# robertknight/ocrs

Hardware: AMD Instinct MI355X
Metric: pages/sec end-to-end (1024x1024) (higher is better)
Workload: dtype f32

## Files before the change

### include/ocrs_amd.h

```cpp
#ifndef OCRS_AMD_H
#define OCRS_AMD_H

#include <stddef.h>
#include <stdint.h>

#if defined(__GNUC__)
#define OCRS_API __attribute__((visibility("default")))
#else
#define OCRS_API
#endif

#ifdef __cplusplus
extern "C" {
#endif

typedef enum ocrs_status {
    OCRS_OK = 0,
    OCRS_ERR_INVALID_ARGUMENT = 1,
    OCRS_ERR_MODEL_NOT_LOADED = 2,
    OCRS_ERR_MODEL_DIMS = 3,
    OCRS_ERR_RUN_FAILED = 4,
    OCRS_ERR_WRONG_OUTPUT = 5,
    OCRS_ERR_IMAGE_SOURCE = 6,
    OCRS_ERR_DEVICE = 7,
    OCRS_ERR_IO = 8,
    OCRS_ERR_CAPACITY = 9
} ocrs_status;

OCRS_API const char* ocrs_last_error(void);

#define OCRS_ABI_VERSION 6u
OCRS_API uint32_t ocrs_abi_version(void);

OCRS_API void ocrs_buffer_free(void* p);

OCRS_API ocrs_status ocrs_device_count(int* n);
OCRS_API ocrs_status ocrs_set_device(int device);
OCRS_API ocrs_status ocrs_get_device(int* device);

OCRS_API ocrs_status ocrs_ctc_beam_search(const float* logp, int t, int c, uint32_t width, int impl, uint32_t** labels,
                                          uint32_t** positions, size_t* n);
OCRS_API ocrs_status ocrs_ctc_beam_search_scored(const float* logp, int t, int c, uint32_t width, int impl, uint32_t** labels,
                                                 uint32_t** positions, size_t* n, double* score, float** step_logp);

OCRS_API ocrs_status ocrs_ctc_decode_packed(const float* logits, const int32_t* lengths, size_t n, int c, const uint8_t* excluded,
                                            int method, uint32_t width, uint32_t** labels, uint32_t** positions,
                                            size_t* step_offsets, float** step_logp, double* scores, float** logp);

OCRS_API ocrs_status ocrs_mask_component_rects(const uint8_t* masks, size_t n, int h, int w, float expand, float min_area,
                                               int max_comp, int64_t arena, int32_t* n_roots, int32_t* overflow, float* rects,
                                               uint8_t* valid);

OCRS_API ocrs_status ocrs_gru_tile_plan(const int32_t* lengths_desc, size_t n_lines, int hidden, int32_t* n_clusters, int32_t* waves,
                                        int16_t* tiles);

OCRS_API ocrs_status ocrs_coalescer_selftest(int n_threads, int requests_per_thread, int max_active, int max_pages,
                                             long window_us, int fail_every, uint64_t out[5]);

OCRS_API ocrs_status ocrs_stream_plan_selftest(int budget, const int32_t* ops, size_t n_ops, int32_t* out);

OCRS_API ocrs_status ocrs_conv_rows_selftest(const float* w, size_t n_w, const float* bias, size_t n_bias, int relu, int y0, int h,
                                             int cin, int32_t out[6]);

OCRS_API ocrs_status ocrs_set_option(const char* name, long value);
OCRS_API ocrs_status ocrs_option_name(int index, const char** name);

OCRS_API ocrs_status ocrs_device_pool_stats(int device, uint64_t out[12]);
OCRS_API ocrs_status ocrs_device_pool_configure(int device, uint64_t device_cached_cap_bytes, uint64_t pinned_cached_cap_bytes);
OCRS_API ocrs_status ocrs_device_pool_trim(int device);

typedef enum { OCRS_ISOLATION_AUTO = 0, OCRS_ISOLATION_NONE = 1 } ocrs_isolation;
OCRS_API ocrs_status ocrs_device_set_isolation(int device, ocrs_isolation policy);
OCRS_API ocrs_status ocrs_device_isolation(int device, int out[3]);

typedef struct ocrs_model ocrs_model;

OCRS_API ocrs_status ocrs_model_load_file(const char* path, ocrs_model** out);
OCRS_API ocrs_status ocrs_model_load_bytes(const void* data, size_t len, ocrs_model** out);
OCRS_API ocrs_status ocrs_model_load_file_on_device(const char* path, int device, ocrs_model** out);
OCRS_API ocrs_status ocrs_model_load_bytes_on_device(const void* data, size_t len, int device, ocrs_model** out);
OCRS_API ocrs_status ocrs_model_device(const ocrs_model* m, int* device);

typedef int (*ocrs_model_run_fn)(void* user, const float* input, const int64_t in_shape[4], float** output,
                                 int64_t out_shape[4], int* out_ndim);
OCRS_API ocrs_status ocrs_model_from_callback(const int64_t input_shape[4],
                                     ocrs_model_run_fn run, void* user, ocrs_model** out);

OCRS_API ocrs_status ocrs_model_input_shape(const ocrs_model* m, int64_t dims[4], uint8_t is_fixed[4]);

typedef struct ocrs_run_options {
    int timing;
} ocrs_run_options;

OCRS_API ocrs_status ocrs_model_run(const ocrs_model* m, const float* input, const int64_t in_shape[4],
                           const ocrs_run_options* opts, float** output, int64_t out_shape[4], int* out_ndim);

OCRS_API ocrs_status ocrs_model_flops(const ocrs_model* m, const int64_t in_shape[4], double* flops);

OCRS_API void ocrs_model_free(ocrs_model* m);

typedef struct ocrs_engine ocrs_engine;
typedef struct ocrs_page ocrs_page;

typedef enum ocrs_numerics { OCRS_NUMERICS_EXACT = 0, OCRS_NUMERICS_RELAXED = 1, OCRS_NUMERICS_REDUCED = 2 } ocrs_numerics;

typedef enum ocrs_decode_method {
    OCRS_DECODE_GREEDY = 0,
    OCRS_DECODE_BEAM_SEARCH = 1
} ocrs_decode_method;

typedef struct ocrs_engine_params {
    const ocrs_model* detection_model;
    const ocrs_model* recognition_model;
    int debug;
    ocrs_decode_method decode_method;
    uint32_t beam_width;
    const char* alphabet;
    const char* allowed_chars;
    ocrs_numerics numerics;
    int coalesce;
    int coalesce_pages;
    int coalesce_window_us;
    int layout_threads;
    int64_t rec_max_pixels;
} ocrs_engine_params;

OCRS_API ocrs_status ocrs_engine_new(const ocrs_engine_params* params, ocrs_engine** out);
OCRS_API void ocrs_engine_free(ocrs_engine* e);
OCRS_API ocrs_status ocrs_engine_device(const ocrs_engine* e, int* device);
OCRS_API ocrs_status ocrs_engine_set_option(ocrs_engine* e, const char* name, long value);
OCRS_API ocrs_status ocrs_engine_get_option(const ocrs_engine* e, const char* name, long* value);

typedef enum ocrs_dim_order { OCRS_HWC = 0, OCRS_CHW = 1 } ocrs_dim_order;
typedef enum ocrs_pixel_type { OCRS_U8 = 0, OCRS_F32 = 1 } ocrs_pixel_type;

OCRS_API ocrs_status ocrs_image_source_check_bytes(size_t len, uint32_t width, uint32_t height, uint32_t* channels);

OCRS_API ocrs_status ocrs_engine_prepare_input(const ocrs_engine* e, const void* pixels, ocrs_pixel_type type,
                                      ocrs_dim_order order, int height, int width, int channels,
                                      ocrs_page** out);
OCRS_API ocrs_status ocrs_engine_prepare_input_batch(const ocrs_engine* e, const void* const* pixels, size_t n,
                                                     ocrs_pixel_type type, ocrs_dim_order order, int height, int width,
                                                     int channels, ocrs_page** out);
OCRS_API ocrs_status ocrs_engine_prepare_input_device(const ocrs_engine* e, const void* d_pixels, ocrs_pixel_type type,
                                             ocrs_dim_order order, int height, int width, int channels,
// ... 381 lines not shown
```

### ocrs_amd/_lib.py

```python
import ctypes as C
import os

_HERE = os.path.dirname(os.path.abspath(__file__))
LIB_PATH = os.environ.get("OCRS_AMD_LIB") or os.path.join(_HERE, "libocrs_amd.so")

OCRS_OK = 0
STATUS_NAMES = {
    0: "OK", 1: "INVALID_ARGUMENT", 2: "MODEL_NOT_LOADED", 3: "MODEL_DIMS", 4: "RUN_FAILED", 5: "WRONG_OUTPUT",
    6: "IMAGE_SOURCE", 7: "DEVICE", 8: "IO", 9: "CAPACITY",
}

RUN_FN = C.CFUNCTYPE(C.c_int, C.c_void_p, C.POINTER(C.c_float), C.POINTER(C.c_int64), C.POINTER(C.POINTER(C.c_float)),
                     C.POINTER(C.c_int64), C.POINTER(C.c_int))


class EngineParams(C.Structure):
    _fields_ = [("detection_model", C.c_void_p), ("recognition_model", C.c_void_p), ("debug", C.c_int),
                ("decode_method", C.c_int), ("beam_width", C.c_uint32), ("alphabet", C.c_char_p),
                ("allowed_chars", C.c_char_p), ("numerics", C.c_int), ("coalesce", C.c_int), ("coalesce_pages", C.c_int),
                ("coalesce_window_us", C.c_int), ("layout_threads", C.c_int), ("rec_max_pixels", C.c_int64)]


class GroupParams(C.Structure):
    _fields_ = [("detection_model", C.c_void_p), ("detection_model_len", C.c_size_t), ("recognition_model", C.c_void_p),
                ("recognition_model_len", C.c_size_t), ("devices", C.POINTER(C.c_int)), ("n_devices", C.c_size_t),
                ("debug", C.c_int), ("decode_method", C.c_int), ("beam_width", C.c_uint32), ("alphabet", C.c_char_p),
                ("allowed_chars", C.c_char_p), ("gather", C.c_int), ("numerics", C.c_int), ("coalesce", C.c_int),
                ("coalesce_pages", C.c_int), ("coalesce_window_us", C.c_int), ("layout_threads", C.c_int), ("rec_max_pixels", C.c_int64),
                ("min_block", C.c_int), ("shared_block", C.c_int)]


class RunOptions(C.Structure):
    _fields_ = [("timing", C.c_int)]


class TextCharC(C.Structure):
    _fields_ = [("ch", C.c_uint32), ("top", C.c_int32), ("left", C.c_int32), ("bottom", C.c_int32),
                ("right", C.c_int32)]


class OcrsError(RuntimeError):
    def __init__(self, status, message):
        super().__init__(message)
        self.status = status
        self.status_name = STATUS_NAMES.get(status, str(status))


DECLARED_SYMBOLS = [
    "ocrs_last_error", "ocrs_buffer_free", "ocrs_device_count", "ocrs_set_device", "ocrs_set_option", "ocrs_ctc_beam_search", "ocrs_model_load_file",
    "ocrs_model_load_bytes", "ocrs_model_from_callback", "ocrs_model_input_shape", "ocrs_model_run",
    "ocrs_model_flops", "ocrs_model_free", "ocrs_engine_new", "ocrs_engine_free", "ocrs_image_source_check_bytes",
    "ocrs_engine_prepare_input", "ocrs_engine_prepare_input_device", "ocrs_page_free", "ocrs_page_dims",
    "ocrs_page_image", "ocrs_engine_detect_words", "ocrs_engine_detect_words_batch",
    "ocrs_engine_detect_text_pixels", "ocrs_engine_detection_threshold", "ocrs_engine_find_text_lines",
    "ocrs_engine_find_text_lines_batch",
    "ocrs_engine_recognize_text", "ocrs_engine_recognize_text_batch", "ocrs_engine_recognize_tokens",
    "ocrs_engine_prepare_recognition_input", "ocrs_text_item_rotated_rect", "ocrs_rotated_rect_corners", "ocrs_engine_get_text", "ocrs_device_malloc", "ocrs_device_free",
    "ocrs_device_upload", "ocrs_device_synchronize", "ocrs_device_measure_peaks", "ocrs_engine_enable_timing", "ocrs_stage_count",
    "ocrs_stage_name", "ocrs_engine_stage_times", "ocrs_kernel_class_count", "ocrs_kernel_class_name",
    "ocrs_engine_kernel_stats", "ocrs_engine_set_kernel_timing_mask", "ocrs_gru_tile_plan", "ocrs_host_malloc", "ocrs_host_free", "ocrs_engine_prepare_input_batch",
    "ocrs_get_device", "ocrs_model_load_file_on_device", "ocrs_model_load_bytes_on_device", "ocrs_model_device", "ocrs_engine_device",
    "ocrs_engine_group_new", "ocrs_engine_group_free", "ocrs_engine_group_size", "ocrs_engine_group_member", "ocrs_group_deal",
    "ocrs_group_prepare_input_batch", "ocrs_group_prepare_input_device_batch", "ocrs_group_detect_words_batch",
    "ocrs_group_recognize_text_batch", "ocrs_group_gather", "ocrs_group_final_gather", "ocrs_group_worker_threads", "ocrs_group_last_gather", "ocrs_device_malloc_on", "ocrs_engine_coalesce_stats", "ocrs_coalescer_selftest", "ocrs_stream_plan_selftest", "ocrs_conv_rows_selftest", "ocrs_engine_kernel_mfma_flops", "ocrs_engine_prepare_input_jpeg", "ocrs_jpeg_decode_rgb", "ocrs_jpeg_info", "ocrs_jpeg_coefficients",
    "ocrs_group_member_stats", "ocrs_numa_parse_cpulist", "ocrs_numa_bind_selftest", "ocrs_engine_recognize_logits", "ocrs_engine_set_option", "ocrs_engine_get_option", "ocrs_option_name", "ocrs_device_pool_stats", "ocrs_device_pool_configure", "ocrs_device_pool_trim",
    "ocrs_device_set_isolation", "ocrs_device_isolation", "ocrs_group_set_replay", "ocrs_abi_version",
    "ocrs_engine_recognize_text_scored", "ocrs_engine_recognize_text_batch_scored", "ocrs_ctc_beam_search_scored",
    "ocrs_engine_run_recognition_ops", "ocrs_ctc_decode_packed", "ocrs_mask_component_rects",
    "ocrs_engine_detect_words_scored", "ocrs_engine_detect_words_batch_scored", "ocrs_group_detect_words_batch_scored",
    "ocrs_engine_find_text_lines_indexed", "ocrs_engine_find_text_lines_batch_indexed",
    "ocrs_detection_tile_plan", "ocrs_engine_detect_words_tiled", "ocrs_engine_detect_words_batch_tiled",
    "ocrs_engine_detect_text_pixels_tiled", "ocrs_group_detect_words_batch_tiled",
    "ocrs_line_frame", "ocrs_line_char_boxes", "ocrs_engine_prepare_recognition_input_rectified",
    "ocrs_engine_recognize_text_rectified", "ocrs_engine_recognize_text_batch_rectified",
    "ocrs_group_recognize_text_batch_rectified", "ocrs_engine_recognize_tokens_rectified",
    "ocrs_engine_rotate_page", "ocrs_engine_rotate_pages", "ocrs_unrotate_rects", "ocrs_unrotate_chars",
    "ocrs_orientation_vote", "ocrs_engine_detect_orientation", "ocrs_engine_page_from_grey",
    "ocrs_engine_resize_page", "ocrs_engine_resize_pages", "ocrs_work_size", "ocrs_rescale_rects",
    "ocrs_engine_detect_words_at", "ocrs_engine_detect_words_batch_at",
    "ocrs_normalize_params_default", "ocrs_normalize_params_check", "ocrs_engine_normalize_page", "ocrs_engine_normalize_pages",
    "ocrs_skew_params_default", "ocrs_skew_params_check", "ocrs_skew_table", "ocrs_engine_skew_scores", "ocrs_engine_estimate_skew",
    "ocrs_engine_warp_page", "ocrs_engine_warp_pages", "ocrs_deskew_map", "ocrs_unwarp_rects", "ocrs_unwarp_chars",
    "ocrs_outline_params_default", "ocrs_outline_params_check", "ocrs_engine_edge_peaks", "ocrs_outline_choose", "ocrs_engine_find_outline",
    "ocrs_quad_map", "ocrs_engine_project_page", "ocrs_engine_project_pages", "ocrs_unproject_rects", "ocrs_unproject_chars",
    "ocrs_rules_params_default", "ocrs_rules_params_check", "ocrs_engine_remove_rules_page", "ocrs_engine_remove_rules_pages",
    "ocrs_speckle_params_default", "ocrs_speckle_params_check", "ocrs_engine_despeckle_page", "ocrs_engine_despeckle_pages",
    "ocrs_binarize_params_default", "ocrs_binarize_params_check", "ocrs_engine_binarize_page", "ocrs_engine_binarize_pages",
]

ABI_VERSION = 6
TILE_OVERLAP_DEFAULT = 100
RESAMPLE_FILTERS = {"auto": 0, "bilinear": 1, "area": 2}
POLARITIES = {"auto": 0, "keep": 1, "invert": 2}


class NormalizeParams(C.Structure):
    _fields_ = [("tile", C.c_int32), ("polarity", C.c_int32), ("flatten", C.c_int32), ("levels", C.c_int32)]


class NormalizeInfo(C.Structure):
    _fields_ = [("dark", C.c_int32), ("white", C.c_int32), ("lo", C.c_int32), ("hi", C.c_int32), ("vote", C.c_int64),
                ("counted", C.c_uint64)]

    def as_dict(self):
        return {"dark": int(self.dark), "vote": int(self.vote), "white": int(self.white), "lo": int(self.lo), "hi": int(self.hi),
                "counted": int(self.counted)}


class RulesParams(C.Structure):
    _fields_ = [("threshold", C.c_float), ("min_length", C.c_int32), ("max_thickness", C.c_int32), ("margin", C.c_int32), ("paper", C.c_float)]


class RulesInfo(C.Structure):
    _fields_ = [("paper_bin", C.c_int32), ("fill", C.c_float), ("ink", C.c_uint64), ("counted", C.c_uint64), ("h_removed", C.c_uint64),
                ("v_removed", C.c_uint64), ("overwritten", C.c_uint64), ("kept", C.c_uint64)]

    def as_dict(self):
        return {"paper_bin": int(self.paper_bin), "fill": float(self.fill), "ink": int(self.ink), "counted": int(self.counted),
                "h_removed": int(self.h_removed), "v_removed": int(self.v_removed), "overwritten": int(self.overwritten),
                "kept": int(self.kept)}


class SpeckleParams(C.Structure):
    _fields_ = [("threshold", C.c_float), ("max_area", C.c_int32), ("max_hole", C.c_int32), ("keep_near", C.c_int32), ("paper", C.c_float),
                ("ink_level", C.c_float)]


class SpeckleInfo(C.Structure):
    _fields_ = [("paper_bin", C.c_int32), ("ink_bin", C.c_int32), ("paper_fill", C.c_float), ("ink_fill", C.c_float), ("ink", C.c_uint64),
                ("counted", C.c_uint64), ("specks", C.c_uint64), ("kept", C.c_uint64), ("speck_pixels", C.c_uint64),
                ("kept_pixels", C.c_uint64), ("holes", C.c_uint64), ("hole_pixels", C.c_uint64)]

    def as_dict(self):
        return {name: (float if name.endswith("_fill") else int)(getattr(self, name)) for name, _ in self._fields_}


class BinarizeParams(C.Structure):
    _fields_ = [("radius", C.c_int32), ("k_q8", C.c_int32), ("keep_ink", C.c_int32), ("ink_level", C.c_float), ("paper", C.c_float)]


class BinarizeInfo(C.Structure):
    _fields_ = [("counted", C.c_uint64), ("ink", C.c_uint64), ("ink_fill", C.c_float), ("paper_fill", C.c_float)]

    def as_dict(self):
        return {name: (float if name.endswith("_fill") else int)(getattr(self, name)) for name, _ in self._fields_}


# ... 247 lines not shown
```

### ocrs_amd/csrc/abi.cpp

```cpp
#include <cstdio>
#include <fstream>
#include <thread>

#include <atomic>
#include "abi_util.hpp"
#include "coalesce_selftest.hpp"
#include "conv_rows.hpp"
#include "engine.hpp"
#include "host_pool.hpp"
#include "jpeg.hpp"
#include "kernels.hpp"
#include "page_ops.hpp"

using namespace ocrs;
using namespace ocrs::geom;

using namespace ocrs::abi;

extern "C" {

const char* ocrs_last_error(void) { return last_error().c_str(); }

void ocrs_buffer_free(void* p) { free(p); }

ocrs_status ocrs_device_count(int* n) {
    return guarded([&] {
        int c = 0;
        hipError_t e = hipGetDeviceCount(&c);
        if (e != hipSuccess) c = 0;
        *n = c;
    });
}

ocrs_status ocrs_set_device(int device) {
    return guarded([&] { select_device(device); });
}

ocrs_status ocrs_get_device(int* device) {
    return guarded([&] {
        if (!device) fail(OCRS_ERR_INVALID_ARGUMENT, "null argument");
        *device = default_device();
    });
}

ocrs_status ocrs_gru_tile_plan(const int32_t* lengths_desc, size_t n_lines, int hidden, int32_t* n_clusters, int32_t* waves,
                               int16_t* tiles) {
    return guarded([&] {
        if (!lengths_desc || !n_clusters || !waves || !tiles || n_lines == 0 || n_lines > (size_t)1 << 20)
            fail(OCRS_ERR_INVALID_ARGUMENT, "bad argument");
        for (size_t i = 0; i < n_lines; i++)
            if (lengths_desc[i] < 1 || (i > 0 && lengths_desc[i] > lengths_desc[i - 1]))
                fail(OCRS_ERR_INVALID_ARGUMENT, "lengths must be positive and descending");
        int ncl = 0;
        if (!k::gru_tile_plan(lengths_desc, (int)n_lines, hidden, &ncl, waves, tiles))
            fail(OCRS_ERR_CAPACITY, "no persistent-kernel plan for this shape (the engine then runs the recurrence as one fused launch per time step)");
        *n_clusters = ncl;
    });
}

ocrs_status ocrs_coalescer_selftest(int n_threads, int requests_per_thread, int max_active, int max_pages, long window_us,
                                    int fail_every, uint64_t out[5]) {
    return guarded([&] {
        if (!out || n_threads < 1 || requests_per_thread < 1 || max_pages < 1) fail(OCRS_ERR_INVALID_ARGUMENT, "bad argument");
        coalescer_selftest(n_threads, requests_per_thread, max_active, max_pages, window_us, fail_every, out);
    });
}

ocrs_status ocrs_stream_plan_selftest(int budget, const int32_t* ops, size_t n_ops, int32_t* out) {
    return guarded([&] {
        if (!out || (n_ops > 0 && !ops) || !LanePlan::valid_budget(budget)) fail(OCRS_ERR_INVALID_ARGUMENT, "bad argument");
        LanePlan plan(budget);
        for (size_t i = 0; i < n_ops; i++) {
            const int32_t op = ops[2 * i], arg = ops[2 * i + 1];
            switch (op) {
                case 0: out[i] = plan.acquire(arg); break;
                case 1: plan.release(arg); out[i] = plan.outstanding(); break;
                case 2: out[i] = plan.set_budget(arg) ? 1 : 0; break;
                case 3: out[i] = plan.load(arg); break;
                case 4: out[i] = plan.budget(); break;
                case 5: out[i] = plan.light_lanes(); break;
                default: fail(OCRS_ERR_INVALID_ARGUMENT, "unknown op %d", (int)op);
            }
        }
    });
}

ocrs_status ocrs_conv_rows_selftest(const float* w, size_t n_w, const float* bias, size_t n_bias, int relu, int y0, int h, int cin,
                                    int32_t out[6]) {
    return guarded([&] {
        if (!out || (n_w > 0 && !w) || (n_bias > 0 && !bias) || h < kConvRowsPatchH || h % kConvRowsPatchH != 0 || y0 < 0 || y0 >= h ||
            y0 % kConvRowsPatchH != 0 || cin < 2 * kConvRowsChunk || cin % (2 * kConvRowsChunk) != 0)
            fail(OCRS_ERR_INVALID_ARGUMENT, "bad argument");
        out[0] = conv_rows_skip_exact(w, n_w, bias, n_bias, relu != 0) ? 1 : 0;
        const RowPhases ph = conv_row_phases(y0, h, cin, out[0] != 0);
        out[1] = ph.c_top;
        out[2] = ph.c_bot;
        for (int phase = 0; phase < 3; phase++) {
            const int c = 3 * phase * (cin / kConvRowsChunk);
            out[3 + phase] = c < ph.c_top ? 0 : c >= ph.c_bot ? kConvRowsPatchH - 1 : -1;
        }
    });
}

namespace {

void beam_search_hook(const float* logp, int t, int c, uint32_t width, int impl, std::vector<uint32_t>* l,
                      std::vector<uint32_t>* p, double* score, std::vector<float>* step_logp) {
    if (impl == 2 && t > 0) {
        DeviceScope bind(-1);
        if (!k::ctc_beam_supported(c, (int)width)) fail(OCRS_ERR_CAPACITY, "beam search on the GPU supports up to 128 classes and width 128");
        Workspace ws;
        std::vector<int32_t> meta(1 + t + 1);
        meta[0] = t;
        for (int i = 0; i <= t; i++) meta[1 + i] = i;
        int32_t* d_meta = ws.alloc_n<int32_t>(meta.size());
        float* d_logp = ws.alloc_n<float>((size_t)t * c);
        ws.upload(d_meta, meta.data(), meta.size() * sizeof(int32_t));
        ws.upload(d_logp, logp, (size_t)t * c * sizeof(float));
        const size_t arena = k::ctc_beam_arena_entries(t, (int)width);
        int2* d_nodes = ws.alloc_n<int2>(arena);
        int2* d_posn = ws.alloc_n<int2>(arena);
        uint32_t* d_ol = ws.alloc_n<uint32_t>(t);
        uint32_t* d_op = ws.alloc_n<uint32_t>(t);
        int32_t* d_cnt = ws.alloc_n<int32_t>(1);
        double* d_score = score ? ws.alloc_n<double>(1) : nullptr;
        float* d_slp = score ? ws.alloc_n<float>(t) : nullptr;
        k::ctc_beam_packed(d_logp, d_meta, d_meta + 1, 1, t, c, (int)width, nullptr, d_nodes, d_posn, d_ol, d_op, d_cnt, ws.s(),
                           d_score, d_slp);
        std::vector<uint32_t> hl(t), hp(t);
        std::vector<float> hs(score ? t : 0);
        int32_t cnt = 0;
        ws.download(hl.data(), d_ol, (size_t)t * 4);
        ws.download(hp.data(), d_op, (size_t)t * 4);
        ws.download(&cnt, d_cnt, 4);
        if (score) {
            ws.download(score, d_score, sizeof(double));
            ws.download(hs.data(), d_slp, (size_t)t * sizeof(float));
        }
        ws.sync();
        OCRS_HIP(hipGetLastError());
        l->assign(hl.begin(), hl.begin() + cnt);
        p->assign(hp.begin(), hp.begin() + cnt);
        if (score) step_logp->assign(hs.begin(), hs.begin() + cnt);
    } else {
        double bs = 0.0;
        const std::vector<CtcStep> st = t == 0 ? std::vector<CtcStep>()
                                              : (impl == 1 ? ctc_beam_search_reference(logp, t, c, c, width, &bs)
                                                           : ctc_beam_search(logp, t, c, c, width, &bs));
        l->resize(st.size()); p->resize(st.size());
        for (size_t i = 0; i < st.size(); i++) { (*l)[i] = st[i].label; (*p)[i] = st[i].pos; }
        if (score) score_line(logp, t, c, c, nullptr, st, &bs, step_logp, score);
    }
}

}

ocrs_status ocrs_ctc_beam_search(const float* logp, int t, int c, uint32_t width, int impl, uint32_t** labels,
                                 uint32_t** positions, size_t* n) {
    return guarded([&] {
        if (!logp || !labels || !positions || !n || t < 0 || c < 1) fail(OCRS_ERR_INVALID_ARGUMENT, "bad argument");
        std::vector<uint32_t> l, p;
        beam_search_hook(logp, t, c, width, impl, &l, &p, nullptr, nullptr);
        *labels = dup_buffer(l);
        *positions = dup_buffer(p);
        *n = l.size();
    });
}

ocrs_status ocrs_ctc_beam_search_scored(const float* logp, int t, int c, uint32_t width, int impl, uint32_t** labels,
                                        uint32_t** positions, size_t* n, double* score, float** step_logp) {
    return guarded([&] {
        if (!logp || !labels || !positions || !n || !score || !step_logp || t < 0 || c < 1)
            fail(OCRS_ERR_INVALID_ARGUMENT, "bad argument");
        std::vector<uint32_t> l, p;
        std::vector<float> s;
        double sc = 0.0;
        beam_search_hook(logp, t, c, width, impl, &l, &p, &sc, &s);
        *labels = dup_buffer(l);
        *positions = dup_buffer(p);
        *step_logp = dup_buffer(s);
        *n = l.size();
        *score = sc;
    });
// ... 998 lines not shown
```

### ocrs_amd/csrc/kernels_rec.hip

```cpp
#include <algorithm>
#include <type_traits>

#include "common.hpp"
#include "conv_rows.hpp"
#include "kernels.hpp"
#include "split_mfma.hpp"

namespace ocrs {
namespace k {

typedef float f32x16 __attribute__((ext_vector_type(16)));
typedef unsigned u32x4 __attribute__((ext_vector_type(4)));
typedef float f32x4 __attribute__((ext_vector_type(4)));
typedef float f32x2 __attribute__((ext_vector_type(2)));
typedef unsigned u32x2 __attribute__((ext_vector_type(2)));
typedef __bf16 bf16x8 __attribute__((ext_vector_type(8)));
typedef __bf16 bf16x2 __attribute__((ext_vector_type(2)));

__device__ __forceinline__ int xcd_remap(int b, int nwg) {
    const int xcd = b & 7, q = nwg >> 3, r = nwg & 7;
    return (xcd < r ? xcd * (q + 1) : r * (q + 1) + (xcd - r) * q) + (b >> 3);
}

__device__ __forceinline__ int find_group(const int32_t* __restrict__ toff, int G, int tile) {
    int lo = 0, hi = G;
    while (hi - lo > 1) {
        int mid = (lo + hi) >> 1;
        if (toff[mid] <= tile) lo = mid; else hi = mid;
    }
    return lo;
}

__global__ void __launch_bounds__(256)
conv1_relu_pool_ragged_kernel(const float* __restrict__ x, RaggedView in, const float* __restrict__ wt,
                              const float* __restrict__ bias, int cout, float* __restrict__ y, RaggedView out) {
    __shared__ float sw[9 * 64 + 64];
    for (int i = threadIdx.x; i < 9 * cout; i += 256) sw[i] = wt[i];
    for (int i = threadIdx.x; i < cout; i += 256) sw[9 * 64 + i] = bias[i];
    __syncthreads();
    const int g = find_group(out.toff256, out.G, blockIdx.x);
    const int tile = blockIdx.x - out.toff256[g];
    const int ow = out.W[g], oh = out.H, iw = in.W[g], ih = in.H;
    const int64_t rows = (int64_t)out.n[g] * oh * ow;
    const float* __restrict__ xg = x + in.poff[g];
    float* __restrict__ yg = y + out.poff[g] * cout;
    const int cq = cout >> 2;
    const int step_px = 256 / cq;
    const int q = threadIdx.x % cq;
    int64_t r = (int64_t)tile * 256 + threadIdx.x / cq;
    int ox = (int)(r % ow);
    int64_t t0 = r / ow;
    int oy = (int)(t0 % oh);
    int64_t img = t0 / oh;
    float wq[9][4], bq[4];
#pragma unroll
    for (int t = 0; t < 9; t++)
#pragma unroll
        for (int c = 0; c < 4; c++) wq[t][c] = sw[t * cout + 4 * q + c];
#pragma unroll
    for (int c = 0; c < 4; c++) bq[c] = sw[9 * 64 + 4 * q + c];
    for (int it = 0; it < cq; it++, r += step_px) {
        if (r >= rows) break;
        if (it > 0) {
            ox += step_px;
            while (ox >= ow) { ox -= ow; if (++oy == oh) { oy = 0; img++; } }
        }
        const float* xi = xg + img * ih * iw;
        float p[4][4];
        const int iy0 = 2 * oy - 1, ix0 = 2 * ox - 1;
        if (iy0 >= 0 && iy0 + 3 < ih && ix0 >= 0 && ix0 + 3 < iw) {
            const float* pp = xi + (int64_t)iy0 * iw + ix0;
#pragma unroll
            for (int a = 0; a < 4; a++)
#pragma unroll
                for (int b = 0; b < 4; b++) p[a][b] = pp[a * iw + b];
        } else {
#pragma unroll
            for (int a = 0; a < 4; a++)
#pragma unroll
                for (int b = 0; b < 4; b++) {
                    const int iy = iy0 + a, ix = ix0 + b;
                    p[a][b] = ((unsigned)iy < (unsigned)ih && (unsigned)ix < (unsigned)iw) ? xi[(int64_t)iy * iw + ix] : 0.0f;
                }
        }
        float m[4];
#pragma unroll
        for (int py = 0; py < 2; py++)
#pragma unroll
            for (int px = 0; px < 2; px++) {
                float acc[4];
#pragma unroll
                for (int c = 0; c < 4; c++) acc[c] = bq[c];
#pragma unroll
                for (int ky = 0; ky < 3; ky++)
// ... 434 lines not shown
                if (soff[it] < 0) continue;
                const int ty = TW == 32 ? 2 * wm + i : 4 * wm + 2 * i + (q >> 4);
                *reinterpret_cast<f32x4*>(&C[soff[it] + (y0 + ty) * Wo * cout]) = *reinterpret_cast<const f32x4*>(&stage[q * WN + sc4]);
            }
            asm volatile("s_waitcnt lgkmcnt(0)" ::: "memory");
        }
        return;
    }
    constexpr int NX = TW == 16 ? 8 : 16;
    int xo_off[FLAT ? NX : 1];
    if (FLAT) {
#pragma unroll
        for (int jx = 0; jx < NX; jx++) {
            if (PW == 2 && (jx & 1)) { xo_off[jx] = -1; continue; }
            const int q = (jx & 3) + 8 * (jx >> 2) + 4 * half_e;
            int x = x0 + (TW == 32 ? q : (q & 15)), ir = 0;
#pragma unroll
            for (int k = 0; k < 3; k++) { const bool nx = x >= Wp; x -= nx ? Wp : 0; ir += nx; }
            xo_off[jx] = (x + (PW - 1) < W && ir < span) ? (ir * Ho * Wo + x / PW) * cout : -1;
        }
    }
    if constexpr (ROWS != 0) {
        const int col = n0 + wave_e * 32 + l31_e;
#pragma unroll
        for (int j = 0; j < 4; j++) {
            if (PH == 2 && (j & 1)) continue;
#pragma unroll
            for (int r = 0; r < 16; r++) {
                if (PW == 2 && (r & 1)) continue;
                const int x = x0 + (r & 3) + 8 * (r >> 2) + 4 * half_e;
                if (FLAT ? xo_off[r] < 0 : x + (PW - 1) >= W) continue;
                const f32x16& a0 = acc[j >> 1][j & 1];
                const f32x16& a1 = acc[(j ^ 1) >> 1][(j ^ 1) & 1];
                float m = act(a0[r]);
                if (PW == 2) { const float v = act(a0[(r + 1) & 15]); m = v > m ? v : m; }
                if (PH == 2) {
                    { const float v = act(a1[r]); m = v > m ? v : m; }
                    if (PW == 2) { const float v = act(a1[(r + 1) & 15]); m = v > m ? v : m; }
                }
                const int yo = (y0 + j) / PH;
                if (FLAT) C[xo_off[r] + yo * Wo * cout + col] = m;
                else C[((int64_t)yo * Wo + x / PW) * cout + col] = m;
            }
        }
        return;
    }
#pragma unroll
    for (int t = 0; t < NTW; t++) {
        const int col = n0 + wn * (BN / 2) + t * 32 + l31;
        if (col >= cout) continue;
#pragma unroll
        for (int i = 0; i < 2; i++) {
            if (PH == 2 && TW == 32 && i == 1) continue;
#pragma unroll
            for (int r = 0; r < 16; r++) {
                if (PH == 2 && TW == 16 && (r & 8)) continue;
                if (PW == 2 && (r & 1)) continue;
                const int q = (r & 3) + 8 * (r >> 2) + 4 * half;
                const int ty = TW == 32 ? 2 * wm + i : 4 * wm + 2 * i + (r >> 3);
                const int tx = TW == 32 ? q : (q & 15);
                const int x = x0 + tx;
                if (FLAT ? xo_off[TW == 16 ? (r & 7) : r] < 0 : x + (PW - 1) >= W) continue;
                constexpr int VI = (PH == 2 && TW == 32) ? 1 : 0;
                constexpr int VR = (PH == 2 && TW == 16) ? 8 : 0;
                float m = act(acc[i][t][r]);
                if (PW == 2) { const float v = act(acc[i][t][(r + 1) & 15]); m = v > m ? v : m; }
                if (PH == 2) {
                    { const float v = act(acc[(i + VI) & 1][t][(r + VR) & 15]); m = v > m ? v : m; }
                    if (PW == 2) { const float v = act(acc[(i + VI) & 1][t][(r + VR + 1) & 15]); m = v > m ? v : m; }
                }
                const int yo = (y0 + ty) / PH;
                if (FLAT) C[xo_off[TW == 16 ? (r & 7) : r] + yo * Wo * cout + col] = m;
                else C[((int64_t)yo * Wo + x / PW) * cout + col] = m;
            }
        }
    }
}

constexpr int F12_MID = 32, F12_COUT = 64, F12_TW = 16, F12_TH = 8, F12_HW = F12_TW + 2, F12_HH = F12_TH + 2;
constexpr int F12_NPOS = F12_HH * F12_HW;
constexpr int F12_LD = F12_MID + 1;
constexpr int F12_BK = 16;
constexpr size_t F12_LDS = (size_t)(F12_NPOS * F12_LD + 2 * F12_BK * F12_COUT) * sizeof(float);

__global__ void __launch_bounds__(256, CONV_WAVES)
conv12_fused_kernel(const float* __restrict__ X0, RaggedView in0, RaggedView mid, const float* __restrict__ w1,
                    const float* __restrict__ b1, const float* __restrict__ Bw, const float* __restrict__ bias,
                    float* __restrict__ Y, const int64_t* __restrict__ out_poff) {
    extern __shared__ __attribute__((aligned(16))) float lds[];
    constexpr int BN = F12_COUT, TW = F12_TW, TH = F12_TH, LD = F12_LD;
    float* T = lds;
    float* Bs = lds + F12_NPOS * LD;
    const int tid = threadIdx.x, lane = tid & 63, wave = tid >> 6;
    const int half = lane >> 5, l31 = lane & 31;
    const int wm = wave >> 1, wn = wave & 1;
    const int gtile = xcd_remap(blockIdx.x, gridDim.x);
    const int g = find_group(mid.toff2d_gap, mid.G, gtile);
    const int tile = gtile - mid.toff2d_gap[g];
    const int H = mid.H, W = mid.W[g];
    const int H0 = in0.H, W0 = in0.W[g];
    const int tiles_h = H / TH;
    const int Wg = (W + 2) & ~1;
    const int nimg = mid.n[g];
    const int rb = tile % tiles_h;
    const int c0 = (tile / tiles_h) * TW;
    const int img = c0 / Wg;
    const int x0 = c0 - img * Wg;
    const int span = min(nimg - img, (x0 + TW - 1) / Wg + 1);
    const int y0 = rb * TH;

    constexpr int BV = F12_BK * BN / 4 / 256;
    const int boff = (tid / (BN / 4)) * BN + (tid % (BN / 4)) * 4;
    auto load_b = [&](int k0, int buf) {
#pragma unroll
        for (int j = 0; j < BV; j++)
            __builtin_amdgcn_global_load_lds((const __attribute__((address_space(1))) void*)(Bw + (int64_t)(k0 + 16 * j) * BN + boff),
                                             (__attribute__((address_space(3))) void*)(Bs + buf * F12_BK * BN + wave * 256 + 1024 * j), 16, 0, 0);
    };
    load_b(0, 0);

    {
        const int q = tid & 7;
        f32x2 wq[9][2], bq[2];
#pragma unroll
        for (int t = 0; t < 9; t++)
#pragma unroll
            for (int c = 0; c < 2; c++) wq[t][c] = f32x2{w1[t * F12_MID + 4 * q + 2 * c], w1[t * F12_MID + 4 * q + 2 * c + 1]};
#pragma unroll
        for (int c = 0; c < 2; c++) bq[c] = f32x2{b1[4 * q + 2 * c], b1[4 * q + 2 * c + 1]};
        const float* __restrict__ xg = X0 + in0.poff[g];
        for (int p = tid >> 3; p < F12_NPOS; p += 32) {
            const int hy = p / F12_HW, hx = p - hy * F12_HW;
            const int y = y0 - 1 + hy;
            int x = x0 - 1 + hx, ir = 0;
#pragma unroll
            for (int k = 0; k < 3; k++) { const bool nx = x >= Wg; x -= nx ? Wg : 0; ir += nx; }
            f32x2 m[2] = {f32x2{0.0f, 0.0f}, f32x2{0.0f, 0.0f}};
            if ((unsigned)y < (unsigned)H && x >= 0 && x < W && ir < span) {
                const float* xi = xg + (int64_t)(img + ir) * H0 * W0;
                float pt[4][4];
                const int iy0 = 2 * y - 1, ix0 = 2 * x - 1;
                if (iy0 >= 0 && iy0 + 3 < H0 && ix0 >= 0 && ix0 + 3 < W0) {
                    const float* pp = xi + (int64_t)iy0 * W0 + ix0;
#pragma unroll
                    for (int a = 0; a < 4; a++)
#pragma unroll
                        for (int b = 0; b < 4; b++) pt[a][b] = pp[a * W0 + b];
                } else {
#pragma unroll
                    for (int a = 0; a < 4; a++)
#pragma unroll
                        for (int b = 0; b < 4; b++) {
                            const int iy = iy0 + a, ix = ix0 + b;
                            pt[a][b] = ((unsigned)iy < (unsigned)H0 && (unsigned)ix < (unsigned)W0) ? xi[(int64_t)iy * W0 + ix] : 0.0f;
                        }
                }
#pragma unroll
                for (int py = 0; py < 2; py++)
#pragma unroll
                    for (int px = 0; px < 2; px++) {
                        f32x2 acc[2] = {bq[0], bq[1]};
#pragma unroll
                        for (int ky = 0; ky < 3; ky++)
#pragma unroll
                            for (int kx = 0; kx < 3; kx++) {
                                const float xs = pt[py + ky][px + kx];
                                const f32x2 xv = f32x2{xs, xs};
#pragma unroll
                                for (int c = 0; c < 2; c++) acc[c] = __builtin_elementwise_fma(xv, wq[ky * 3 + kx][c], acc[c]);
                            }
#pragma unroll
                        for (int c = 0; c < 2; c++) m[c] = (py == 0 && px == 0) ? acc[c] : __builtin_elementwise_max(acc[c], m[c]);
                    }
#pragma unroll
                for (int c = 0; c < 2; c++) {
                    m[c].x = m[c].x > 0.0f ? m[c].x : 0.0f;
                    m[c].y = m[c].y > 0.0f ? m[c].y : 0.0f;
                }
            }
            float* t = T + p * LD + 4 * q;
            t[0] = m[0].x; t[1] = m[0].y; t[2] = m[1].x; t[3] = m[1].y;
        }
    }

    f32x16 acc[2];
    {
        const int col = wn * 32 + l31;
        const float bv = bias[col];
#pragma unroll
        for (int r = 0; r < 16; r++) { acc[0][r] = bv; acc[1][r] = bv; }
    }
    int abase[2];
#pragma unroll
    for (int i = 0; i < 2; i++) {
        const int m = wm * 64 + i * 32 + l31;
        abase[i] = ((m / TW) * F12_HW + (m % TW)) * LD + half;
    }
    __syncthreads();
    constexpr int NCH = 9 * F12_MID / F12_BK;
    static_assert(F12_MID % F12_BK == 0 && F12_BK % 16 == 0, "chunk size");
#pragma unroll
    for (int c = 0; c < NCH; c++) {
        if (c + 1 < NCH) load_b((c + 1) * F12_BK, (c + 1) & 1);
        const int tap = (c * F12_BK) / F12_MID, ch0 = (c * F12_BK) % F12_MID;
        const int toff = ((tap / 3) * F12_HW + tap % 3) * LD + ch0;
        const float* b = Bs + (c & 1) * F12_BK * BN + wn * 32 + l31;
#pragma unroll
        for (int kp = 0; kp < F12_BK / 2; kp++) {
            const float a0 = T[abase[0] + toff + 2 * kp], a1 = T[abase[1] + toff + 2 * kp];
            const float bt = b[(2 * kp + half) * BN];
            acc[0] = __builtin_amdgcn_mfma_f32_32x32x2f32(a0, bt, acc[0], 0, 0, 0);
            acc[1] = __builtin_amdgcn_mfma_f32_32x32x2f32(a1, bt, acc[1], 0, 0, 0);
        }
        __syncthreads();
    }

    const int Ho = H / 2, Wo = W / 2;
    float* __restrict__ C = Y + (out_poff[g] + (int64_t)img * Ho * Wo) * BN;
    auto act = [&](float v) { return v > 0.0f ? v : 0.0f; };
    const int col = wn * 32 + l31;
    int xo_off[8];
#pragma unroll
    for (int jx = 0; jx < 8; jx++) {
        if (jx & 1) { xo_off[jx] = -1; continue; }
        int x = x0 + (jx & 3) + 8 * (jx >> 2) + 4 * half, ir = 0;
#pragma unroll
        for (int k = 0; k < 3; k++) { const bool nx = x >= Wg; x -= nx ? Wg : 0; ir += nx; }
        xo_off[jx] = (x + 1 < W && ir < span) ? (ir * Ho * Wo + x / 2) * BN : -1;
    }
#pragma unroll
    for (int i = 0; i < 2; i++)
#pragma unroll
        for (int r = 0; r < 8; r += 2) {
            if (xo_off[r & 7] < 0) continue;
            const float m = act(__builtin_fmaxf(__builtin_fmaxf(acc[i][r], acc[i][r + 1]), __builtin_fmaxf(acc[i][r + 8], acc[i][r + 9])));
            const int yo = (y0 + 4 * wm + 2 * i) / 2;
            C[xo_off[r & 7] + yo * Wo * BN + col] = m;
        }
}

constexpr int F12S_RS = 20;
constexpr int F12S_TILE = F12_HH * F12S_RS * 64;
constexpr int F12S_BTAP = F12_COUT * 64;
constexpr size_t f12s_lds(int np) { return (size_t)np * (F12S_TILE + 3 * F12S_BTAP); }

template <int NP>
__global__ void __launch_bounds__(256, NP == 3 ? 2 : 3)
conv12_fused_split_kernel(const float* __restrict__ X0, RaggedView in0, RaggedView mid, const float* __restrict__ w1,
                          const float* __restrict__ b1, const uint16_t* __restrict__ Bimg, const float* __restrict__ bias,
                          float* __restrict__ Y, const int64_t* __restrict__ out_poff) {
    extern __shared__ __attribute__((aligned(16))) float lds[];
    constexpr int BN = F12_COUT, TW = F12_TW, TH = F12_TH;
    char* T = reinterpret_cast<char*>(lds);
    char* Bs = T + NP * F12S_TILE;
    const int tid = threadIdx.x, lane = tid & 63, wave = tid >> 6;
    const int half = lane >> 5, l31 = lane & 31;
    const int wm = wave >> 1, wn = wave & 1;
    const int gtile = xcd_remap(blockIdx.x, gridDim.x);
    const int g = find_group(mid.toff2d_gap, mid.G, gtile);
    const int tile = gtile - mid.toff2d_gap[g];
    const int H = mid.H, W = mid.W[g];
    const int H0 = in0.H, W0 = in0.W[g];
    const int tiles_h = H / TH;
    const int Wg = (W + 2) & ~1;
    const int nimg = mid.n[g];
    const int rb = tile % tiles_h;
// ... 316 lines not shown
```

Before: 286.9.

## Compute fused conv1 stage with MFMA over an LDS-staged pixel window

Replaces the scalar FMA implementation of the first 3x3 conv plus 2x2 maxpool inside the fused conv12 kernel with 32x32x1 f32 MFMA instructions. The input pixel window is first staged into the second weight buffer in LDS, and pooling is done from accumulator registers. Boundary validity moves to ballot-built row and column masks. Launch bounds change to 5 blocks per CU. The aim is to cut VALU cost in stage 1, at the price of new LDS window loads, an extra barrier, and different register pressure. It also adds a selftest ABI entry describing the tile mapping.

```diff
diff --git a/include/ocrs_amd.h b/include/ocrs_amd.h
--- a/include/ocrs_amd.h
+++ b/include/ocrs_amd.h
@@ -61,6 +61,8 @@
 
 OCRS_API ocrs_status ocrs_conv_rows_selftest(const float* w, size_t n_w, const float* bias, size_t n_bias, int relu, int y0, int h,
                                              int cin, int32_t out[6]);
+
+OCRS_API ocrs_status ocrs_conv12_mfma_selftest(int32_t dims[6], int32_t rows[96], int32_t acc_rows[128], int32_t taps[18]);
 
 OCRS_API ocrs_status ocrs_set_option(const char* name, long value);
 OCRS_API ocrs_status ocrs_option_name(int index, const char** name);
diff --git a/ocrs_amd/_lib.py b/ocrs_amd/_lib.py
--- a/ocrs_amd/_lib.py
+++ b/ocrs_amd/_lib.py
@@ -62,7 +62,7 @@
     "ocrs_get_device", "ocrs_model_load_file_on_device", "ocrs_model_load_bytes_on_device", "ocrs_model_device", "ocrs_engine_device",
     "ocrs_engine_group_new", "ocrs_engine_group_free", "ocrs_engine_group_size", "ocrs_engine_group_member", "ocrs_group_deal",
     "ocrs_group_prepare_input_batch", "ocrs_group_prepare_input_device_batch", "ocrs_group_detect_words_batch",
-    "ocrs_group_recognize_text_batch", "ocrs_group_gather", "ocrs_group_final_gather", "ocrs_group_worker_threads", "ocrs_group_last_gather", "ocrs_device_malloc_on", "ocrs_engine_coalesce_stats", "ocrs_coalescer_selftest", "ocrs_stream_plan_selftest", "ocrs_conv_rows_selftest", "ocrs_engine_kernel_mfma_flops", "ocrs_engine_prepare_input_jpeg", "ocrs_jpeg_decode_rgb", "ocrs_jpeg_info", "ocrs_jpeg_coefficients",
+    "ocrs_group_recognize_text_batch", "ocrs_group_gather", "ocrs_group_final_gather", "ocrs_group_worker_threads", "ocrs_group_last_gather", "ocrs_device_malloc_on", "ocrs_engine_coalesce_stats", "ocrs_coalescer_selftest", "ocrs_stream_plan_selftest", "ocrs_conv_rows_selftest", "ocrs_conv12_mfma_selftest", "ocrs_engine_kernel_mfma_flops", "ocrs_engine_prepare_input_jpeg", "ocrs_jpeg_decode_rgb", "ocrs_jpeg_info", "ocrs_jpeg_coefficients",
     "ocrs_group_member_stats", "ocrs_numa_parse_cpulist", "ocrs_numa_bind_selftest", "ocrs_engine_recognize_logits", "ocrs_engine_set_option", "ocrs_engine_get_option", "ocrs_option_name", "ocrs_device_pool_stats", "ocrs_device_pool_configure", "ocrs_device_pool_trim",
     "ocrs_device_set_isolation", "ocrs_device_isolation", "ocrs_group_set_replay", "ocrs_abi_version",
     "ocrs_engine_recognize_text_scored", "ocrs_engine_recognize_text_batch_scored", "ocrs_ctc_beam_search_scored",
diff --git a/ocrs_amd/csrc/abi.cpp b/ocrs_amd/csrc/abi.cpp
--- a/ocrs_amd/csrc/abi.cpp
+++ b/ocrs_amd/csrc/abi.cpp
@@ -5,6 +5,7 @@
 #include <atomic>
 #include "abi_util.hpp"
 #include "coalesce_selftest.hpp"
+#include "conv12_mfma.hpp"
 #include "conv_rows.hpp"
 #include "engine.hpp"
 #include "host_pool.hpp"
@@ -99,6 +100,24 @@
             const int c = 3 * phase * (cin / kConvRowsChunk);
             out[3 + phase] = c < ph.c_top ? 0 : c >= ph.c_bot ? kConvRowsPatchH - 1 : -1;
         }
+    });
+}
+
+ocrs_status ocrs_conv12_mfma_selftest(int32_t dims[6], int32_t rows[96], int32_t acc_rows[128], int32_t taps[18]) {
+    return guarded([&] {
+        if (!dims || !rows || !acc_rows || !taps) fail(OCRS_ERR_INVALID_ARGUMENT, "bad argument");
+        const int32_t d[6] = {kC12Pairs, kC12TilePos, kC12Taps, kC12HaloH, kC12HaloW, kC12Mid};
+        std::copy_n(d, 6, dims);
+        for (int m = 0; m < 32; m++) {
+            const C12Row r = conv12_tile_row(m);
+            rows[3 * m] = r.u; rows[3 * m + 1] = r.py; rows[3 * m + 2] = r.px;
+        }
+        for (int half = 0; half < 2; half++)
+            for (int r = 0; r < 32; r++) {
+                const C12Acc a = conv12_acc_row(r, half);
+                acc_rows[2 * (32 * half + r)] = a.block; acc_rows[2 * (32 * half + r) + 1] = a.row;
+            }
+        for (int t = 0; t < kC12Taps; t++) { taps[2 * t] = conv12_tap(t).ky; taps[2 * t + 1] = conv12_tap(t).kx; }
     });
 }
 
diff --git a/ocrs_amd/csrc/conv12_mfma.hpp b/ocrs_amd/csrc/conv12_mfma.hpp
--- /dev/null
+++ b/ocrs_amd/csrc/conv12_mfma.hpp
@@ -0,0 +1,23 @@
+#pragma once
+
+namespace ocrs {
+
+constexpr int kC12Mid = 32;
+constexpr int kC12HaloW = 18, kC12HaloH = 10;
+constexpr int kC12Pos = kC12HaloH * kC12HaloW;
+constexpr int kC12TilePos = 8;
+constexpr int kC12Pairs = 12;
+constexpr int kC12Taps = 9;
+constexpr int kC12WinW = 2 * kC12HaloW + 2, kC12WinH = 2 * kC12HaloH + 2;
+static_assert(2 * kC12Pairs * kC12TilePos >= kC12Pos && (2 * kC12Pairs - 2) * kC12TilePos < kC12Pos, "pairs cover the halo");
+
+struct C12Row { int u, py, px; };
+constexpr C12Row conv12_tile_row(int m) { return C12Row{m >> 2, (m >> 1) & 1, m & 1}; }
+
+struct C12Acc { int block, row; };
+constexpr C12Acc conv12_acc_row(int r, int half) { return C12Acc{r >> 4, (r & 3) + 8 * ((r >> 2) & 3) + 4 * half}; }
+
+struct C12Tap { int ky, kx; };
+constexpr C12Tap conv12_tap(int t) { return C12Tap{t / 3, t % 3}; }
+
+}
diff --git a/ocrs_amd/csrc/kernels_rec.hip b/ocrs_amd/csrc/kernels_rec.hip
--- a/ocrs_amd/csrc/kernels_rec.hip
+++ b/ocrs_amd/csrc/kernels_rec.hip
@@ -2,6 +2,7 @@
 #include <type_traits>
 
 #include "common.hpp"
+#include "conv12_mfma.hpp"
 #include "conv_rows.hpp"
 #include "kernels.hpp"
 #include "split_mfma.hpp"
@@ -10,6 +11,7 @@
 namespace k {
 
 typedef float f32x16 __attribute__((ext_vector_type(16)));
+typedef float f32x32 __attribute__((ext_vector_type(32)));
 typedef unsigned u32x4 __attribute__((ext_vector_type(4)));
 typedef float f32x4 __attribute__((ext_vector_type(4)));
 typedef float f32x2 __attribute__((ext_vector_type(2)));
@@ -610,8 +612,15 @@
 constexpr int F12_LD = F12_MID + 1;
 constexpr int F12_BK = 16;
 constexpr size_t F12_LDS = (size_t)(F12_NPOS * F12_LD + 2 * F12_BK * F12_COUT) * sizeof(float);
-
-__global__ void __launch_bounds__(256, CONV_WAVES)
+constexpr int F12_WW = kC12WinW, F12_WH = kC12WinH;
+static_assert(F12_MID == kC12Mid && F12_HW == kC12HaloW && F12_HH == kC12HaloH, "conv12_mfma.hpp describes this kernel's stage 1");
+static_assert(F12_WW * F12_WH <= F12_BK * F12_COUT, "the pixel window must fit weight buffer 1");
+static_assert(5 * F12_LDS <= 160 * 1024, "five blocks per CU");
+static_assert(conv12_acc_row(4, 0).row == 8 && conv12_acc_row(0, 1).row == 4 && conv12_acc_row(19, 1).row == 7 &&
+              conv12_acc_row(19, 1).block == 1 && kC12TilePos == 8,
+              "accumulator registers 16 b + 4 g .. + 3 of a lane are rows 4 (2 g + half) .. + 3 of block b: one position's pooling window");
+
+__global__ void __launch_bounds__(256, 5)
 conv12_fused_kernel(const float* __restrict__ X0, RaggedView in0, RaggedView mid, const float* __restrict__ w1,
                     const float* __restrict__ b1, const float* __restrict__ Bw, const float* __restrict__ bias,
                     float* __restrict__ Y, const int64_t* __restrict__ out_poff) {
@@ -647,69 +656,71 @@
     };
     load_b(0, 0);
 
+    float* Wn = Bs + F12_BK * BN;
+    auto load_window = [&] {
+        const float* __restrict__ xg = X0 + in0.poff[g] + (int64_t)img * H0 * W0;
+        const int Wg2 = 2 * Wg;
+        for (int e = tid; e < F12_WH * F12_WW; e += 256) {
+            const int r = e / F12_WW, c = e - r * F12_WW;
+            const int iy = 2 * y0 - 3 + r;
+            int ix = 2 * x0 - 3 + c, ir = 0;
+#pragma unroll
+            for (int k = 0; k < 3; k++) { const bool nx = ix >= Wg2; ix -= nx ? Wg2 : 0; ir += nx; }
+            float v = 0.0f;
+            if ((unsigned)iy < (unsigned)H0 && (unsigned)ix < (unsigned)W0 && ir < span) v = xg[((int64_t)ir * H0 + iy) * W0 + ix];
+            Wn[e] = v;
+        }
+    };
+
     {
-        const int q = tid & 7;
-        f32x2 wq[9][2], bq[2];
-#pragma unroll
-        for (int t = 0; t < 9; t++)
-#pragma unroll
-            for (int c = 0; c < 2; c++) wq[t][c] = f32x2{w1[t * F12_MID + 4 * q + 2 * c], w1[t * F12_MID + 4 * q + 2 * c + 1]};
-#pragma unroll
-        for (int c = 0; c < 2; c++) bq[c] = f32x2{b1[4 * q + 2 * c], b1[4 * q + 2 * c + 1]};
-        const float* __restrict__ xg = X0 + in0.poff[g];
-        for (int p = tid >> 3; p < F12_NPOS; p += 32) {
-            const int hy = p / F12_HW, hx = p - hy * F12_HW;
-            const int y = y0 - 1 + hy;
-            int x = x0 - 1 + hx, ir = 0;
+        const int wave_s = __builtin_amdgcn_readfirstlane(wave);
+        float wb[kC12Taps];
+#pragma unroll
+        for (int t = 0; t < kC12Taps; t++) wb[t] = w1[t * F12_MID + l31];
+        const float bv1 = b1[l31];
+        const C12Row row = conv12_tile_row(l31);
+        unsigned colmask, rowmask;
+        {
+            int x = x0 - 1 + lane, ir = 0;
 #pragma unroll
             for (int k = 0; k < 3; k++) { const bool nx = x >= Wg; x -= nx ? Wg : 0; ir += nx; }
-            f32x2 m[2] = {f32x2{0.0f, 0.0f}, f32x2{0.0f, 0.0f}};
-            if ((unsigned)y < (unsigned)H && x >= 0 && x < W && ir < span) {
-                const float* xi = xg + (int64_t)(img + ir) * H0 * W0;
-                float pt[4][4];
-                const int iy0 = 2 * y - 1, ix0 = 2 * x - 1;
-                if (iy0 >= 0 && iy0 + 3 < H0 && ix0 >= 0 && ix0 + 3 < W0) {
-                    const float* pp = xi + (int64_t)iy0 * W0 + ix0;
-#pragma unroll
-                    for (int a = 0; a < 4; a++)
-#pragma unroll
-                        for (int b = 0; b < 4; b++) pt[a][b] = pp[a * W0 + b];
-                } else {
-#pragma unroll
-                    for (int a = 0; a < 4; a++)
-#pragma unroll
-                        for (int b = 0; b < 4; b++) {
-                            const int iy = iy0 + a, ix = ix0 + b;
-                            pt[a][b] = ((unsigned)iy < (unsigned)H0 && (unsigned)ix < (unsigned)W0) ? xi[(int64_t)iy * W0 + ix] : 0.0f;
-                        }
+            colmask = (unsigned)__builtin_amdgcn_ballot_w64(lane < F12_HW && x >= 0 && x < W && ir < span);
+            rowmask = (unsigned)__builtin_amdgcn_ballot_w64(lane < F12_HH && (unsigned)(y0 - 1 + lane) < (unsigned)H);
+        }
+        load_window();
+#pragma unroll
+        for (int t = 0; t < kC12Taps; t++) asm volatile("" : "+v"(wb[t]));
+        __syncthreads();
+        for (int pair = wave_s; pair < kC12Pairs; pair += 4) {
+            const int ap = min((2 * pair + half) * kC12TilePos + row.u, F12_NPOS - 1);
+            const int ahy = ap / F12_HW, ahx = ap - ahy * F12_HW;
+            const float* a = Wn + (2 * ahy + row.py) * F12_WW + 2 * ahx + row.px;
+            f32x32 c1;
+#pragma unroll
+            for (int r = 0; r < 32; r++) c1[r] = bv1;
+#pragma unroll
+            for (int t = 0; t < kC12Taps; t++)
+                c1 = __builtin_amdgcn_mfma_f32_32x32x1f32(a[conv12_tap(t).ky * F12_WW + conv12_tap(t).kx], wb[t], c1, 0, 0, 0);
+#pragma unroll
+            for (int b = 0; b < 2; b++) {
+                const int p0 = (2 * pair + b) * kC12TilePos, hy0 = p0 / F12_HW, hx0 = p0 - hy0 * F12_HW;
+#pragma unroll
+                for (int gq = 0; gq < 4; gq++) {
+                    if (p0 + 2 * gq >= F12_NPOS) continue;
+                    int phx = hx0 + 2 * gq + half, phy = hy0;
+                    if (phx >= F12_HW) { phx -= F12_HW; phy++; }
+                    float m = c1[16 * b + 4 * gq];
+                    m = __builtin_fmaxf(c1[16 * b + 4 * gq + 1], m);
+                    m = __builtin_fmaxf(c1[16 * b + 4 * gq + 2], m);
+                    m = __builtin_fmaxf(c1[16 * b + 4 * gq + 3], m);
+                    m = m > 0.0f ? m : 0.0f;
+                    const bool inside = ((colmask >> phx) & (rowmask >> phy) & 1u) != 0;
+                    T[(p0 + 2 * gq + half) * LD + l31] = inside ? m : 0.0f;
                 }
-#pragma unroll
-                for (int py = 0; py < 2; py++)
-#pragma unroll
-                    for (int px = 0; px < 2; px++) {
-                        f32x2 acc[2] = {bq[0], bq[1]};
-#pragma unroll
-                        for (int ky = 0; ky < 3; ky++)
-#pragma unroll
-                            for (int kx = 0; kx < 3; kx++) {
-                                const float xs = pt[py + ky][px + kx];
-                                const f32x2 xv = f32x2{xs, xs};
-#pragma unroll
-                                for (int c = 0; c < 2; c++) acc[c] = __builtin_elementwise_fma(xv, wq[ky * 3 + kx][c], acc[c]);
-                            }
-#pragma unroll
-                        for (int c = 0; c < 2; c++) m[c] = (py == 0 && px == 0) ? acc[c] : __builtin_elementwise_max(acc[c], m[c]);
-                    }
-#pragma unroll
-                for (int c = 0; c < 2; c++) {
-                    m[c].x = m[c].x > 0.0f ? m[c].x : 0.0f;
-                    m[c].y = m[c].y > 0.0f ? m[c].y : 0.0f;
-                }
-            }
-            float* t = T + p * LD + 4 * q;
-            t[0] = m[0].x; t[1] = m[0].y; t[2] = m[1].x; t[3] = m[1].y;
-        }
-    }
+            }
+        }
+    }
+
 
     f32x16 acc[2];
     {
```

Result: no change. 285.3 (-0.5%).
